# motionlife/gqmap-opticalflow

Hardware: AMD Instinct MI355X
Metric: Gpixel-iters/s + AEPE vs .flo GT, Middlebury 584x388, 1/2/4/8 GPU (higher is better)
Workload: dtype f64; 1 GPU; C2: rubberwhale 584x388 mixture L=1 K=9 its=2541 (one step = one full-frame iteration); engine=mixture, L=1, K=9, parallelism=frame-parallel x1

## Files before the change

gqmap-opticalflow_amd/csrc/gqmap_engine.hip:

```cpp
#include <dlfcn.h>
#include <hip/hip_runtime.h>
#include <rccl/rccl.h>

#include <algorithm>
#include <chrono>
#include <condition_variable>
#include <cstdlib>
#include <cmath>
#include <cstring>
#include <mutex>
#include <string>
#include <vector>

#include "gqmap_internal.h"
#include "gqmap_blockmatch.h"

#pragma clang fp contract(off)

namespace gq {
__device__ __forceinline__ double gq_sqrt_dev(double x)
{
    const double y = __builtin_amdgcn_rsq(x);
    double g = x * y, h = 0.5 * y;
    const double r = fma(-h, g, 0.5);
// ... 70 lines not shown
}
#define GQ_ROOT_STAGED 1

#define GQ_HD __device__ __forceinline__
#define GQ_SQRT(x) gq::gq_sqrt_dev(x)
#include "gqmap_tuning.h"
#define GQ_STR2(x) #x
#define GQ_PRAGMA_UNROLL(n) _Pragma(GQ_STR2(unroll n))
#define GQ_UNROLL2 GQ_PRAGMA_UNROLL(GQ_EDGE_UNROLL_N)
#define GQ_PAIR_UNROLL GQ_PRAGMA_UNROLL(GQ_PAIR_UNROLL_N)
#define GQ_PAIR_UNROLL_K(n) GQ_PRAGMA_UNROLL(n)
#define GQ_NODE_UNROLL GQ_PRAGMA_UNROLL(GQ_NODE_UNROLL_N)
#define GQ_UNROLL_FULL _Pragma("unroll")
#define GQ_UMUL24(a, b) __umul24((uint32_t)(a), (uint32_t)(b))
#define GQ_FRACT(x) __builtin_amdgcn_fract(x)
#include "gqmap_math.h"

namespace gq {

typedef float vvs_t;

constexpr int TILE = 16;
constexpr int BLOCK = TILE * TILE;
constexpr int TS = TAB_STRIDE;
constexpr int NPLANES = 9;
constexpr int TRACE_CAP = 8192;
constexpr int GRAPH_CHUNK = 50;
#ifndef GQ_FLOW_CHUNK
#define GQ_FLOW_CHUNK 250
#endif
// ... 589 lines not shown
        for (int x = 0; x < ACC_SLICES; ++x) t += v[x];
#pragma unroll
        for (int x = 0; x < ACC_SLICES; ++x) __hip_atomic_store(a + x * SL, 0ull, __ATOMIC_RELAXED, __HIP_MEMORY_SCOPE_AGENT);
        sh[tid] = t;
    }
    __syncthreads();
    if (tid < NP) {
        fix128 v = 0;
#pragma unroll
        for (int k = 3; k >= 0; --k) v = (v << 32) + (fix128)(long long)sh[4 * tid + k];
        out[tid] = v;
    }
    if (tid == 0) ctl->arrive = 0;
}

template <typename R, typename VT, int ENG, int Q, bool EDGE_FIRST, bool COH = false, bool NT = false,
          bool LIT = false, bool GRP = false, int ROTF = GQ_NODE_ROT_OTHER, int HALO = 0>
__device__ __forceinline__ void iter_tile(const IterParams<R, VT> P, int tile, int it, int parity,
                                          int part_r, TileLdsQ<R, Q> &lds, int l0, int l1, double Tcur,
                                          bool tab_ready, unsigned long long *acc_ring = nullptr,
                                          int grows = 0, bool grouped = false, HaloChain<R> *hc = nullptr,
                                          unsigned halo_tok = 0
#if GQ_FLOW_TL
                                          , unsigned long long *tlw = nullptr
#endif
                                          )
{
    static_assert(HALO == 0 || (GRP && sizeof(R) == 8), "the halo forms: the fp64 dataflow item (one component per item)");
    constexpr bool CHAIN = HALO == 1;
    static_assert(!LIT || (ENG == 0 && Q == 1 && sizeof(R) == 8), "literal order: fp64 mixture, Q = 1");
    static_assert(!GRP || (Q == 1 && !LIT), "a tile per wave: one lane per node");
    constexpr bool RS = Q == 0;
    constexpr int QA = arith_q(Q);
    constexpr int TPIX = tile_pix(Q);
    constexpr int TM = tile_rows(Q), TN = TPIX / TM;
    static_assert(TM * TN == TPIX, "tile");
    Ctl *ctl = P.ctl;
// ... 66 lines not shown
        R eE = 0, eda = 0;
#pragma unroll
        for (int ph = 0; ph < 2; ++ph) {
        if ((ph == 0) != EDGE_FIRST) {
        if (do_node && LIT) {
            if constexpr (LIT)
                if (inner)
                    nd = lit_node_grad(tab, K2, P.VV, P.M2, P.I1, P.Mo, P.No, P.epsn, P.lamd, P.guard != 0, T, a,
                                       mu_u, mu_v, sg_u, sg_v, pn, m, n + P.n_off);
        } else if (do_node) {
        NodeCoef<R> c{};
        if (inner) c = node_coef(sg_u, sg_v, pn);
        const bool fast = ENG == 0 && __all(!inner || node_unclamped(c, mu_u, mu_v, m, n + P.n_off, P.Mo, P.No,
                                                                     P.gh_xmax, R(ENG == 2 ? CTF_MARGIN : 0.0)));
        if (inner) {
            const auto fv = frame_view(P.VV, P.M2);
            constexpr bool PF = QA >= GQ_NODE_PF_MIN_Q && (QA > 1 || sizeof(VT) == 4);
            constexpr int ROT = PF ? ROTF : 0;
            Sums<R> S = fast ? node_sums<ENG, false, PF, ROT>(tab, kj, K2, QA, fv, P.I1, P.Mo, P.No, P.epsn, c, mu_u,
                                                              mu_v, m, n + P.n_off)
                             : node_sums<ENG, true, PF, ROT>(tab, kj, K2, QA, fv, P.I1, P.Mo, P.No, P.epsn, c, mu_u,
                                                             mu_v, m, n + P.n_off);
            if (QA > 1) S = lane_combine<QA>(S);
            nd = node_epi(S, c, P.lamd, P.guard != 0, T, a, sg_u, sg_v, pn, ENG == 2);
            if constexpr (RS) {
                lds.nd[0][pix] = nd.du1; lds.nd[1][pix] = nd.du2; lds.nd[2][pix] = nd.do1;
                lds.nd[3][pix] = nd.do2; lds.nd[4][pix] = nd.dp; lds.nd[5][pix] = nd.E; lds.nd[6][pix] = nd.da;
            }
        }
        }
        } else if (do_edge) {
// ... 685 lines not shown
void k_iter_flow(IterParams<R, VT> P, int n_iter, unsigned *fl, int ntiles, const Ctl *snap)
{
    static_assert(Q >= 1 && Q <= 4, "1..4 lanes per node");
    static_assert(!LIT || (ENG == 0 && Q == 1), "literal order: the mixture engine at one lane per node");
    unsigned *bar = P.bar;
    const bool run = !snap->stop && __hip_atomic_load(&P.ctl->stop, __ATOMIC_RELAXED, __HIP_MEMORY_SCOPE_AGENT) == 0 &&
                     __hip_atomic_load(bar + BAR_FAIL, __ATOMIC_RELAXED, __HIP_MEMORY_SCOPE_AGENT) == 0;
    const int it0 = snap->it, done0 = snap->done;
    const double T0 = snap->T;
    const int b = blockIdx.x, xcd = b & 7;
    int s0 = 0;
    for (int y = 0; y < xcd; ++y) s0 += (ntiles - y + 7) >> 3;
    const int nb = (ntiles - xcd + 7) >> 3;
    const int L = ENG == 1 ? P.L : 1, nitems = ntiles * L;
    constexpr bool GRP = GQ_FLOW_GROUPS && Q == 1 && !LIT && (ENG == 0 || ENG == 2);
    constexpr int ROTF = ENG == 0 && Q == 1 && !LIT && W == 0 && sizeof(R) == 8 && is_vvh2<VT>::value
                             ? (GQ_NODE_ROT_FLOW_FP64 | NODE_UNROLL(GQ_NODE_UNROLL_FLOW_FP64))
                             : GQ_NODE_ROT_OTHER;
    constexpr int HALO = !GRP || LIT || W != 0 || sizeof(R) != 8 ? 0
                         : ENG == 0 && is_vvh2<VT>::value ? GQ_FLOW_HALO
                         : ENG == 2 ? GQ_FLOW_HALO_CTF : 0;
    HaloChain<R> *hc = nullptr;
    if constexpr (HALO == 1) {
        __shared__ HaloChain<R> sh_halo;
        hc = &sh_halo;
        if (threadIdx.x < 4) sh_halo.flag[threadIdx.x] = 0;
        if (threadIdx.x == 0) sh_halo.fail = bar + BAR_FAIL;
    }
    const int vr = P.M - (P.tiles_m - 1) * tile_rows(Q);
    const bool groups = GRP && GQ_FLOW_ROWS && vr <= 4;
    const int nlast = groups ? (s0 + nb) / P.tiles_m - s0 / P.tiles_m : 0;
    const int nbl = groups ? nb - nlast + ((nlast + 3) >> 2) : nb * L;
    constexpr int INV = ENG == 2 && Q == 1 ? GQ_PHASE_MIX_CTF_Q1_INV : GQ_PHASE_MIX_OTHER_INV;
    constexpr bool MIX = GQ_FLOW_MIX && ENG == 0 && (!LIT || GQ_FLOW_LIT_MIX);
    const bool edge_first = MIX && ((((b >> 3) / P.cu_slots) & 1) != INV);
    __shared__ TileLdsQ<R, Q> lds;
    __shared__ int sh_i, sh_go, sh_last;
    __shared__ int sh_grp[4];
    __shared__ double tot[NFIX + GQMAP_LMAX];
    __shared__ unsigned long long sh_acc[4 * (NFIX + GQMAP_LMAX)];
    unsigned long long *acc = reinterpret_cast<unsigned long long *>(fl + FL_ACC);
    unsigned *q = fl + FL_Q + xcd * FL_LINE;
// ... 46 lines not shown
            for (int q = 0; q < nd; ++q) T = fmax(T * P.fin.drate, P.fin.t_min);
        }
        unsigned long long *slot = acc + (size_t)(j % FL_SLOTS) * FL_ACC_SLOT;
        const int l0 = ENG == 1 ? l : 0, l1 = ENG == 1 ? l + 1 : 1;
        const int wtile = GRP ? __builtin_amdgcn_readfirstlane(grouped ? sh_grp[threadIdx.x >> 6] : tile) : tile;
        const int wrows = grouped ? vr : tile_rows(Q);
#if GQ_FLOW_TL
        const size_t tlwi = (size_t)j * nitems + (size_t)tile * L + l;
        unsigned long long *tlw = (tlwi + 1) * 16 <= (size_t)(4 * FLOW_TL_WORDS) && snap->it == 1 ? g_flow_tlw + tlwi * 16 : nullptr;
#define GQ_TLW_ARG , tlw
#else
#define GQ_TLW_ARG
#endif
        if (MIX && edge_first)
            iter_tile<R, VT, ENG, Q, true, GQ_FLOW_COH, false, LIT, GRP, ROTF, HALO>(P, wtile, it, parity, 0, lds, l0, l1, T, false, slot,
                                                                                wrows, grouped, hc, (unsigned)i + 1 GQ_TLW_ARG);
        else
            iter_tile<R, VT, ENG, Q, false, GQ_FLOW_COH, false, LIT, GRP, ROTF, HALO>(P, wtile, it, parity, 0, lds, l0, l1, T, false, slot,
                                                                                 wrows, grouped, hc, (unsigned)i + 1 GQ_TLW_ARG);
#undef GQ_TLW_ARG
        asm volatile("s_waitcnt vmcnt(0)" ::: "memory");
        __syncthreads();
#if GQ_FLOW_TL
        const size_t tli = (size_t)j * nitems + (size_t)tile * L + l;
        if (threadIdx.x == 0 && (tli + 1) * 4 <= (size_t)FLOW_TL_WORDS && snap->it == 1) {
            unsigned long long *w = g_flow_tl + tli * 4;
            w[0] = tl_claim;
            w[1] = tl_go;
            w[2] = __builtin_amdgcn_s_memrealtime();
            w[3] = ((unsigned long long)__builtin_amdgcn_s_getreg((31 << 11) | 20) << 32) |
                   (unsigned)__builtin_amdgcn_s_getreg((31 << 11) | 4);
        }
#endif
        if (GRP && grouped && threadIdx.x > 0 && (int)threadIdx.x < gsize)
// ... 302 lines not shown

namespace gq {
struct Policy {
    int nt_state = -1;
    int band_rows = -1;
    int cu_group = -1;
    int lpar = -1;
    int lpar_xcd = 1;
    int fused_finalize = 1;
    int persist = 1;
    int persist_cap = -1;
    int graph = 1;
    int flow = -1;
    int vv_float = 1;
    int vv_pair = 1;
    int verbose = 0;
};
Policy g_pol;
}

struct gqmap_ctx {
    gqmap_options opt;
    int device = 0;
    hipStream_t stream = nullptr;
    bool fp32 = false, super_ = false;
    int Mo = 0, No = 0, M = 0, N = 0, L = 0, K = 0, K2 = 0;
    int64_t MNL = 0;
    size_t rsz = 8;
    void *d_VV = nullptr, *d_I1 = nullptr, *d_st[2] = {nullptr, nullptr}, *d_tab = nullptr;
    Ctl *d_ctl = nullptr;
// ... 3 lines not shown
    Ctl *d_snap_ctl = nullptr;
    size_t snap_bytes = 0;
    bool persist_off = false;
    double *d_trace = nullptr;
    Ctl *h_ctl = nullptr;
    double *h_ring = nullptr;
    unsigned *h_fail = nullptr;
    int ctl_it = 0;
    bool ctl_known = false;
    double *d_truth = nullptr;
    size_t truth_elems = 0;
    int tiles_m = 0, tiles_n = 0, nblocks = 0;
    bool have_images = false, have_state = false;
    bool vv32 = false;
    bool vvp = false;
    bool lit = false;
    int split = 1;
    int kq = 1;
    int lpar = 1;
    hipGraphExec_t graph = nullptr;
    hipGraphExec_t sub[6] = {nullptr, nullptr, nullptr, nullptr, nullptr, nullptr};
    bool own_stream = true;
    double tab_host[NTAB * TS];
    int n_tiles = 1, tile = 0, Ng = 0, col0 = 0, col1 = 0, n_off = 0, own_lo = 0, own_hi = 0;
    int nranks = 0;
    fix128 *d_gathered = nullptr;
    bool own_gathered = false;
    void *d_halo[4] = {nullptr, nullptr, nullptr, nullptr};
    struct RcclComm *comm = nullptr;
    bool in_group = false;
// ... 127 lines not shown
    if (c->pol.band_rows >= 0) return c->pol.band_rows == 1;
    const size_t vsz = c->fp32 ? sizeof(float) : c->vvp ? sizeof(vvh2_t) : c->vv32 ? sizeof(vvs_t) : sizeof(double);
    return vv_elems(c->Mo, c->No) * vsz > ((size_t)4 << 20);
}

bool fused_finalize(const gqmap_ctx *c)
{
    return c->nranks == 0 && c->pol.fused_finalize;
}

template <typename R, typename VT>
IterParams<R, VT> iter_params(const gqmap_ctx *c)
{
    IterParams<R, VT> P;
    const gqmap_options &o = c->opt;
    P.VV = (const VT *)c->d_VV;
    P.I1 = (const R *)c->d_I1;
    P.st0 = (R *)c->d_st[0];
    P.st1 = (R *)c->d_st[1];
    P.tab = (const R *)c->d_tab;
    P.ctl = c->d_ctl;
    P.partials = c->d_partials;
    P.M = c->M; P.N = c->N; P.Mo = c->Mo; P.No = c->No; P.M2 = c->Mo + 2;
    P.L = c->L; P.K2 = c->K2;
    P.tiles_m = c->tiles_m; P.tiles_n = c->tiles_n;
    P.seg_lo[0] = P.seg_lo[1] = 0;
    P.seg_n[0] = c->tiles_m * c->tiles_n;
    P.seg_n[1] = 0;
    P.part_off = 0;
    P.epsn = R(o.epsn); P.lamd = R(o.lambdad); P.lams = R(o.lambdas);
    P.minu = R(o.minu); P.maxu = R(o.maxu); P.minv = R(o.minv); P.maxv = R(o.maxv);
// ... 692 lines not shown
        }
        if (hipMemsetAsync(c->d_flow, 0, sizeof(unsigned) * flow_words(nitems), c->stream) != hipSuccess ||
            hipStreamSynchronize(c->stream) != hipSuccess)
            return false;
        c->flow_n = flow_words(nitems);
    }
    if (!ensure_snap(c)) return false;
    if (dry) return true;
    {
        const int64_t nv = (int64_t)c->MNL * NPLANES;
        const int grid = (int)std::min<int64_t>((nv + 255) / 256, 512);
        k_persist_snap<R><<<grid, 256, 0, c->stream>>>(c->d_ctl, c->d_bar, (const R *)c->d_st[0],
                                                       (const R *)c->d_st[1], (R *)c->d_snap, c->d_snap_ctl, nv);
    }
    IterParams<R, VT> P = iter_params<R, VT>(c);
    if constexpr (ENG == 0 && Q == 1 && !LIT) {
        if (nitems > GQ_FLOW_WIDE_ITEMS) {
            flow_launch<R, VT, ENG, Q, LIT, 3>(c, P, n, nitems, ntiles);
            return true;
        }
    }
    flow_launch<R, VT, ENG, Q, LIT, 0>(c, P, n, nitems, ntiles);
    return true;
}

template <typename R, typename VT>
bool launch_flow_t(gqmap_ctx *c, int n, bool dry)
{
    if (c->opt.engine == GQMAP_ENGINE_SUPER) {
        if constexpr (sizeof(R) == 8) return c->pol.flow > 0 && c->kq == 4 && launch_flow_q<R, VT, 1, 4>(c, n, dry);
        return false;
// ... 13 lines not shown
        default: return false;
        }
    }
    return false;
}

bool launch_flow(gqmap_ctx *c, int n, bool dry)
{
    const bool on = c->pol.flow > 0 || (c->pol.flow < 0 && !c->fp32);
    if (!on || c->persist_off || (c->L != 1 && c->opt.engine != GQMAP_ENGINE_SUPER) || c->n_tiles != 1 ||
        c->comm || c->nranks != 0 || !fused_finalize(c) || n < 1)
        return false;
    if (c->fp32)
        return c->vvp ? !c->lit && c->kq == 1 && launch_flow_q<float, vvh2_t, 0, 1>(c, n, dry)
                      : launch_flow_t<float, float>(c, n, dry);
    if (c->vvp) return !c->lit && c->kq == 1 && launch_flow_q<double, vvh2_t, 0, 1>(c, n, dry);
    if (c->vv32) return launch_flow_t<double, vvs_t>(c, n, dry);
    return launch_flow_t<double, double>(c, n, dry);
}

gqmap_status persist_recover(gqmap_ctx *c, bool *recovered)
{
    *recovered = false;
    if (!c->d_snap) return GQMAP_OK;
    c->ctl_known = false;
    unsigned f = 0;
    GQ_HIP(hipMemcpyAsync(&f, c->d_bar + BAR_FAIL, sizeof(f), hipMemcpyDeviceToHost, c->stream));
    GQ_HIP(hipStreamSynchronize(c->stream));
    if (f == 0) return GQMAP_OK;
    Ctl h;
// ... 174 lines not shown
    strip_geometry(c, Mo, No);
    tile_grid(c);
    if (vvp && (c->kq != 1 || c->split != 1)) {
        vvp = false;
        vv32 = true;
    }
    const bool resize = geom || vv32 != c->vv32 || vvp != c->vvp || !c->d_VV;
    c->vv32 = vv32;
    c->vvp = vvp;
    if (resize) {
        drop_graph(c);
        GQ_HIP(hipStreamSynchronize(c->stream));
        if (c->d_VV) (void)hipFree(c->d_VV);
        if (c->d_I1) (void)hipFree(c->d_I1);
        c->d_VV = c->d_I1 = nullptr;
        if (c->d_truth) (void)hipFree(c->d_truth);
        c->d_truth = nullptr;
        c->truth_elems = 0;
        const size_t vsz = c->fp32 ? sizeof(float) : vvp ? sizeof(vvh2_t) : vv32 ? sizeof(vvs_t) : sizeof(double);
        GQ_HIP(hipMalloc(&c->d_VV, vv_elems(Mo, No) * vsz));
        GQ_HIP(hipMemsetAsync(c->d_VV, 0, vv_elems(Mo, No) * vsz, c->stream));
        GQ_HIP(hipMalloc(&c->d_I1, (size_t)Mo * No * c->rsz));
        gqmap_status s = alloc_grid(c);
        if (s != GQMAP_OK) return s;
        c->have_state = false;
        if (c->n_tiles > 1) {
            for (int k = 0; k < 4; ++k) {
                if (c->d_halo[k]) (void)hipFree(c->d_halo[k]);
                c->d_halo[k] = nullptr;
                GQ_HIP(hipMalloc(&c->d_halo[k], halo_bytes(c, k)));
// ... 244 lines not shown
    gqmap_status s = prepare_images(c, Mo, No, vv32, vvp);
    if (s != GQMAP_OK) return s;
    vvp = c->vvp;
    vv32 = c->vv32;
    DeviceGuard dg(c->device);
    if (vvp) {
        const size_t M2 = (size_t)Mo + 2, N2 = (size_t)No + 2;
        std::vector<vvh2_t> vp(VV.size());
        for (size_t cc = 0; cc < N2; ++cc)
            for (size_t r = 0; r < M2; ++r) {
                vp[r + M2 * cc].lo = (_Float16)VV[r + M2 * cc];
                vp[r + M2 * cc].hi = cc + 1 < N2 ? (_Float16)VV[r + M2 * (cc + 1)] : (_Float16)0;
            }
        GQ_HIP(hipMemcpyAsync(c->d_VV, vp.data(), vp.size() * sizeof(vvh2_t), hipMemcpyHostToDevice, c->stream));
        GQ_HIP(hipStreamSynchronize(c->stream));
    } else if (vv32 && !c->fp32) {
        std::vector<vvs_t> vc(VV.size());
        for (size_t k = 0; k < VV.size(); ++k) vc[k] = (vvs_t)VV[k];
        GQ_HIP(hipMemcpyAsync(c->d_VV, vc.data(), vc.size() * sizeof(vvs_t), hipMemcpyHostToDevice, c->stream));
        GQ_HIP(hipStreamSynchronize(c->stream));
    } else if (vv32) {
        std::vector<float> v32(VV.begin(), VV.end());
        GQ_HIP(hipMemcpyAsync(c->d_VV, v32.data(), v32.size() * sizeof(float), hipMemcpyHostToDevice, c->stream));
        GQ_HIP(hipStreamSynchronize(c->stream));
    } else if ((s = upload(c, c->d_VV, VV.data(), VV.size())) != GQMAP_OK) {
        return s;
    }
    if ((s = upload(c, c->d_I1, I1, (size_t)Mo * No)) != GQMAP_OK) return s;
    c->have_images = true;
    return GQMAP_OK;
// ... 453 lines not shown
}

int gqmap_debug_flow_chunk(void) { return FLOW_CHUNK; }

int gqmap_debug_policy(const char *name, int value)
{
    if (!name) return -1;
    struct Field { const char *n; int *p; int dflt; };
    const Field fields[] = {
        {"nt_state", &g_pol.nt_state, -1},   {"band_rows", &g_pol.band_rows, -1},
        {"cu_group", &g_pol.cu_group, -1},   {"lpar", &g_pol.lpar, -1},
        {"lpar_xcd", &g_pol.lpar_xcd, 1},    {"fused_finalize", &g_pol.fused_finalize, 1},
        {"persist", &g_pol.persist, 1},      {"persist_cap", &g_pol.persist_cap, -1},
        {"graph", &g_pol.graph, 1},          {"vv_float", &g_pol.vv_float, 1}, {"vv_pair", &g_pol.vv_pair, 1},
        {"verbose", &g_pol.verbose, 0},      {"flow", &g_pol.flow, -1},
    };
    for (const Field &f : fields)
        if (std::strcmp(f.n, name) == 0) {
            *f.p = value == -1 ? f.dflt : value;
            return 0;
        }
    return -1;
}

gqmap_status gqmap_get_info(gqmap_ctx *c, gqmap_info *info)
{
    clear_error();
    GQ_CHECK(c && info, GQMAP_ERR_INVALID_ARG, "null argument");
    DeviceGuard dg(c->device);
    std::memset(info, 0, sizeof(*info));
// ... 125 lines not shown
        GQ_HIP(hipMemcpyAsync(out, c->d_VV, nvv * sizeof(double), hipMemcpyDeviceToHost, c->stream));
        GQ_HIP(hipStreamSynchronize(c->stream));
        return GQMAP_OK;
    }
    const size_t esz = c->fp32 ? sizeof(float) : sizeof(vvs_t);
    std::vector<unsigned char> raw(nvv * esz);
    GQ_HIP(hipMemcpyAsync(raw.data(), c->d_VV, raw.size(), hipMemcpyDeviceToHost, c->stream));
    GQ_HIP(hipStreamSynchronize(c->stream));
    for (size_t k = 0; k < nvv; ++k) {
        if (c->fp32) out[k] = ((const float *)raw.data())[k];
        else out[k] = (double)((const vvs_t *)raw.data())[k];
    }
    return GQMAP_OK;
}

gqmap_status gqmap_synchronize(gqmap_ctx *c)
{
    clear_error();
    GQ_CHECK(c, GQMAP_ERR_INVALID_ARG, "null context");
    DeviceGuard dg(c->device);
    GQ_HIP(hipStreamSynchronize(c->stream));
    return GQMAP_OK;
}

gqmap_status gqmap_create_tile(gqmap_ctx **out, const gqmap_options *opt, int device, int n_tiles, int tile)
{
    clear_error();
    GQ_CHECK(n_tiles >= 1 && n_tiles <= 1024, GQMAP_ERR_INVALID_ARG, "n_tiles=%d outside [1,1024]", n_tiles);
    GQ_CHECK(tile >= 0 && tile < n_tiles, GQMAP_ERR_INVALID_ARG, "tile %d of %d", tile, n_tiles);
    gqmap_status s = gqmap_create(out, opt, device);
// ... 282 lines not shown
void gqmap_destroy(gqmap_ctx *c)
{
    if (!c) return;
    DeviceGuard dg(c->device);
    if (c->stream) (void)hipStreamSynchronize(c->stream);
    drop_graph(c);
    if (c->comm) {
        if (c->comm->comm) (void)rccl()->CommDestroy(c->comm->comm);
        delete c->comm;
    }
    for (void *p : {(void *)c->d_rows, (void *)c->d_seqg})
        if (p) (void)hipFree(p);
    if (c->own_gathered && c->d_gathered) (void)hipFree(c->d_gathered);
    for (void *p : c->d_halo)
        if (p) (void)hipFree(p);
    void *bufs[] = {c->d_VV, c->d_I1, c->d_st[0], c->d_st[1], c->d_tab, c->d_ctl, (void *)c->d_partials, c->d_trace,
                    c->d_truth, (void *)c->d_bar, c->d_snap, (void *)c->d_snap_ctl, (void *)c->d_flow};
    for (void *p : bufs)
        if (p) (void)hipFree(p);
    for (void *p : {(void *)c->h_ctl, (void *)c->h_ring, (void *)c->h_fail})
        if (p) (void)hipHostFree(p);
    if (c->stream && c->own_stream) (void)hipStreamDestroy(c->stream);
    delete c;
}

}
```

gqmap-opticalflow_amd/csrc/gqmap_math.h:

```cpp
#pragma once
#include <stdint.h>
#include <string.h>

#include <type_traits>

namespace gq {

#ifndef GQ_M_PI
#define GQ_M_PI 3.14159265358979323846
#define GQ_M_SQRT2 1.41421356237309504880
#endif

constexpr int TAB_STRIDE = 256;
constexpr int NTAB = 8;
constexpr int T_XI = 0, T_XJ = 1, T_W = 2, T_WA = 3, T_WXI = 4, T_WXJ = 5, T_WM = 6, T_WX = 7;
#ifdef __HIPCC__
__host__ __device__
#endif
constexpr int tab_at(int r, int k) { return k * NTAB + r; }

GQ_HD uint64_t bits_of(double x)
{
    uint64_t u;
    memcpy(&u, &x, 8);
// ... 120 lines not shown
GQ_HD VP elem_ptr(VP VV, uint32_t elem)
{
    return byte_ptr(VV, elem * (uint32_t)sizeof(*VV));
}

#if defined(__HIPCC__)
struct alignas(4) vvh2_t {
    _Float16 lo, hi;
};
template <typename T>
struct is_vvh2 : std::is_same<typename std::remove_cv<T>::type, vvh2_t> {};
#else
template <typename T>
struct is_vvh2 : std::false_type {};
#endif
template <typename R, typename E>
GQ_HD R tap_col(const E &e, int half)
{
#if defined(__HIPCC__)
    if constexpr (is_vvh2<E>::value) return R((float)(half ? e.hi : e.lo));
    else
#endif
    {
        (void)half;
        return R(e);
    }
}

template <typename R, typename VP>
GQ_HD R bicubic_w4(VP VV, uint32_t o, uint32_t M2, R s0, R s1, R s2, R s3, R t0, R t1, R t2, R t3)
// ... 30 lines not shown
    keys4(so, s0, s1, s2, s3);
    return bicubic_w4<R>(VV, o, M2, s0, s1, s2, s3, t0, t1, t2, t3);
}

template <typename E>
struct Taps16 {
    E v[16];
};
template <typename VP>
GQ_HD auto load_taps16(VP VV, uint32_t o, uint32_t M2)
{
    using E = typename std::remove_cv<typename std::remove_reference<decltype(*VV)>::type>::type;
    constexpr uint32_t EB = (uint32_t)sizeof(E);
    const uint32_t ob = o * EB, cb = M2 * EB;
    Taps16<E> T;
    if constexpr (is_vvh2<E>::value) {
        for (int pr = 0; pr < 2; ++pr) {
            const auto col = byte_ptr(VV, ob + (uint32_t)(2 * pr) * cb);
            for (int r = 0; r < 4; ++r) T.v[4 * pr + r] = col[r];
        }
        return T;
    } else {
        for (int c = 0; c < 4; ++c) {
            const auto col = byte_ptr(VV, ob + (uint32_t)c * cb);
            for (int r = 0; r < 4; ++r) T.v[4 * c + r] = col[r];
        }
        return T;
    }
}
template <typename R, typename E>
GQ_HD R bicubic_taps4(const Taps16<E> &T, R so, R to)
// ... 47 lines not shown
    return fma(s3, v[3], fma(s2, v[2], fma(s1, v[1], s0 * v[0])));
}

GQ_HD uint32_t cell_elem(int iy, int ix, int M2) { return (uint32_t)(iy - 1) + GQ_UMUL24(M2, ix - 1); }

template <typename VP>
struct TapView {
    VP p;
    uint32_t ld;
    GQ_HD uint32_t cell(int iy, int ix) const { return cell_elem(iy, ix, (int)ld); }
};
template <typename VP>
GQ_HD TapView<VP> frame_view(VP VV, int M2)
{
    return TapView<VP>{VV, (uint32_t)M2};
}

constexpr int VV_TAIL = 8;
constexpr size_t vv_elems(int Mo, int No) { return (size_t)(Mo + 2) * (size_t)(No + 3) + VV_TAIL; }

template <bool CLAMP = true>
GQ_HD void axis_cell_abs(double X, int n, int &ix, double &fr)
{
    if (CLAMP) X = fmin(fmax(X, 1.0), (double)n);
    ix = (int)X;
    fr = GQ_FRACT(X);
}
template <bool CLAMP = true>
GQ_HD void axis_cell(int j, double x, int n, int &ix, double &fr)
{
// ... 372 lines not shown
    R s, t, ax, bx, ay, by;
};
template <typename R>
GQ_HD NodeCoef<R> node_coef(R o1, R o2, R p)
{
    NodeCoef<R> c;
    spectral_st(p, c.s, c.t);
    const R sq2 = R(GQ_M_SQRT2);
    c.ax = sq2 * o1 * c.s; c.bx = sq2 * o1 * c.t;
    c.ay = sq2 * o2 * c.t; c.by = sq2 * o2 * c.s;
    return c;
}
constexpr int NODE_ROT = 1, NODE_ROT_STAGE = 2, NODE_ROT_FLAGS = 255;
constexpr int NODE_UNROLL(int n) { return n << 8; }
constexpr int node_rot_unroll(int rot) { return (rot >> 8) > 1 ? (rot >> 8) : 1; }
template <int ENG, bool CLAMP = true, bool PF = false, int ROT = 0, typename R, typename TP, typename TV, typename IP>
GQ_HD Sums<R> node_sums(TP tab, int k0, int K2, int dk, const TV &V, IP I1, int Mo, int No,
                        R eps, const NodeCoef<R> &c, R u1, R u2, int m, int n)
{
    Sums<R> S;
    if constexpr (PF && ENG != 1) {
        const R I = I1[m + (int64_t)Mo * n];
        constexpr bool ABS = ENG == 0 && sizeof(R) == 8;
        const R U1 = ABS ? u1 + R(n + 1) : u1, U2 = ABS ? u2 + R(m + 1) : u2;
        auto locate = [&](int k, R &so, R &to) -> uint32_t {
            const R x1 = fma(c.ax, tab[tab_at(T_XI, k)], fma(c.bx, tab[tab_at(T_XJ, k)], U1));
            const R x2 = fma(c.ay, tab[tab_at(T_XI, k)], fma(c.by, tab[tab_at(T_XJ, k)], U2));
            if constexpr (ABS) return cell4_abs_v<CLAMP>(V, Mo, No, (double)x1, (double)x2, so, to);
            else if constexpr (ENG == 2) return cell_ctf4_v<CLAMP>(V, Mo, No, m + 1, n + 1, x1, x2, so, to);
            else return cell4_v<CLAMP>(V, Mo, No, m + 1, n + 1, x1, x2, so, to);
        };
        if constexpr ((ROT & NODE_ROT_FLAGS) != 0) {
            static_assert(ROT & NODE_ROT, "the other bits modify the rotated loop");
            constexpr bool STAGE = (ROT & NODE_ROT_STAGE) != 0;
            constexpr int UNR = node_rot_unroll(ROT);
            (void)UNR;
// ... 30 lines not shown
            R so, to;
            auto T = load_taps16(V.p, locate(k0, so, to), V.ld);
            constexpr int UNR = node_rot_unroll(ROT);
            (void)UNR;
            GQ_PAIR_UNROLL_K(UNR)
            for (int k = k0; k <= klast; k += dk) {
                const auto Tk = T;
                const R sok = so, tok = to;
                const int kn = k + dk <= klast ? k + dk : klast;
                T = load_taps16(V.p, locate(kn, so, to), V.ld);
                const R d = fma(bicubic_taps4<R>(Tk, sok, tok), R(-0.25), I);
                S.add(tab, k, GQ_SQRT(fma(d, d, eps)));
            }
        }
        return S;
    }
    if constexpr (ENG != 1) {
        const R I = I1[m + (int64_t)Mo * n];
        if constexpr (ENG == 0 && sizeof(R) == 8) {
            const R U1 = u1 + R(n + 1), U2 = u2 + R(m + 1);
            GQ_NODE_UNROLL
            for (int k = k0; k < K2; k += dk) {
                const R X = fma(c.ax, tab[tab_at(T_XI, k)], fma(c.bx, tab[tab_at(T_XJ, k)], U1));
                const R Y = fma(c.ay, tab[tab_at(T_XI, k)], fma(c.by, tab[tab_at(T_XJ, k)], U2));
                const R d = fma(sample4_abs_v<CLAMP>(V, Mo, No, X, Y), R(-0.25), I);
                S.add(tab, k, GQ_SQRT(fma(d, d, eps)));
            }
        } else {
            GQ_NODE_UNROLL
            for (int k = k0; k < K2; k += dk) {
                const R x1 = fma(c.ax, tab[tab_at(T_XI, k)], fma(c.bx, tab[tab_at(T_XJ, k)], u1));
                const R x2 = fma(c.ay, tab[tab_at(T_XI, k)], fma(c.by, tab[tab_at(T_XJ, k)], u2));
// ... 424 lines not shown
```

gqmap-opticalflow_amd/csrc/gqmap_tuning.h:

```cpp
#pragma once

#ifndef GQ_EDGE_UNROLL_N
#define GQ_EDGE_UNROLL_N 2
#endif
#ifndef GQ_PAIR_UNROLL_N
#define GQ_PAIR_UNROLL_N 2
#endif
#ifndef GQ_PAIR_UNROLL_Q1
#define GQ_PAIR_UNROLL_Q1 4
#endif
#ifndef GQ_NODE_UNROLL_N
#define GQ_NODE_UNROLL_N 1
#endif
#ifndef GQ_FIN_GROUP
#define GQ_FIN_GROUP 1
#endif
#ifndef GQ_EDGE_PK
#define GQ_EDGE_PK 1
#endif
#ifndef GQ_TAB_LDS
#define GQ_TAB_LDS 1
#endif
#ifndef GQ_PHASE_MIX
#define GQ_PHASE_MIX 1
// ... 31 lines not shown
#ifndef GQ_FLOW_HALO
#define GQ_FLOW_HALO 1
#endif
#ifndef GQ_FLOW_HALO_CTF
#define GQ_FLOW_HALO_CTF 1
#endif
#ifndef GQ_FLOW_HALO_ROT_WAVE
#define GQ_FLOW_HALO_ROT_WAVE 2
#endif
#ifndef GQ_FLOW_HALO_EPI
#define GQ_FLOW_HALO_EPI 8
#endif
#ifndef GQ_FLOW_HALO_SLEEP
#define GQ_FLOW_HALO_SLEEP 1
#endif
#ifndef GQ_UNROLL_MIN_Q
#define GQ_UNROLL_MIN_Q 2
#endif
#ifndef GQ_PERSIST_Q4
#define GQ_PERSIST_Q4 0
#endif
#ifndef GQ_PERSIST_SLEEP
#define GQ_PERSIST_SLEEP 2
#endif
#ifndef GQ_TIMELINE
#define GQ_TIMELINE 0
#endif
```

Before: 1.788 Gpixel-iter/s.

## Store frame taps as 16-bit LDS offsets into a per-block value LUT

When the frame pixel values are integers within a small range, the flow kernel stores each tap as a uint16 byte offset into a shared-memory table of doubles instead of half-precision pairs. Each bicubic tap is then resolved by an LDS load, and a dedicated pipelined node-sum loop uses scheduling fences and register pins to overlap the next tap fetch with the current arithmetic. The aim is to reduce the cost of tap fetch and conversion in the fp64 mixture node loop. In exchange it adds per-block LUT fill, extra LDS pressure, a second device buffer and host preprocessing, and it disables the wide-item variant on this path.

```diff
diff --git a/gqmap-opticalflow_amd/csrc/gqmap_engine.hip b/gqmap-opticalflow_amd/csrc/gqmap_engine.hip
--- a/gqmap-opticalflow_amd/csrc/gqmap_engine.hip
+++ b/gqmap-opticalflow_amd/csrc/gqmap_engine.hip
@@ -108,6 +108,11 @@
 #define GQ_UNROLL_FULL _Pragma("unroll")
 #define GQ_UMUL24(a, b) __umul24((uint32_t)(a), (uint32_t)(b))
 #define GQ_FRACT(x) __builtin_amdgcn_fract(x)
+#define GQ_LDS_AS __attribute__((address_space(3)))
+#define GQ_LUT_AT(lut, o) (*(const GQ_LDS_AS double *)((const GQ_LDS_AS char *)(lut) + (o)))
+#define GQ_SCHED_FENCE __builtin_amdgcn_sched_barrier(0)
+#define GQ_PIN64(x) asm volatile("" : "+v"(x))
+#define GQ_PIN_UNIFORM(x) asm volatile("" : "+s"(x))
 #include "gqmap_math.h"
 
 namespace gq {
@@ -727,13 +732,24 @@
     if (tid == 0) ctl->arrive = 0;
 }
 
+template <typename R, typename VT>
+__device__ __forceinline__ auto tile_frame_view(const IterParams<R, VT> &P, const GQ_LDS_AS double *taplut)
+{
+    if constexpr (is_vvo2<VT>::value) {
+        return frame_view_lut(P.VV, P.M2, taplut);
+    } else {
+        (void)taplut;
+        return frame_view(P.VV, P.M2);
+    }
+}
+
 template <typename R, typename VT, int ENG, int Q, bool EDGE_FIRST, bool COH = false, bool NT = false,
           bool LIT = false, bool GRP = false, int ROTF = GQ_NODE_ROT_OTHER, int HALO = 0>
 __device__ __forceinline__ void iter_tile(const IterParams<R, VT> P, int tile, int it, int parity,
                                           int part_r, TileLdsQ<R, Q> &lds, int l0, int l1, double Tcur,
                                           bool tab_ready, unsigned long long *acc_ring = nullptr,
                                           int grows = 0, bool grouped = false, HaloChain<R> *hc = nullptr,
-                                          unsigned halo_tok = 0
+                                          unsigned halo_tok = 0, const GQ_LDS_AS double *taplut = nullptr
 #if GQ_FLOW_TL
                                           , unsigned long long *tlw = nullptr
 #endif
@@ -830,7 +846,7 @@
         const bool fast = ENG == 0 && __all(!inner || node_unclamped(c, mu_u, mu_v, m, n + P.n_off, P.Mo, P.No,
                                                                      P.gh_xmax, R(ENG == 2 ? CTF_MARGIN : 0.0)));
         if (inner) {
-            const auto fv = frame_view(P.VV, P.M2);
+            const auto fv = tile_frame_view(P, taplut);
             constexpr bool PF = QA >= GQ_NODE_PF_MIN_Q && (QA > 1 || sizeof(VT) == 4);
             constexpr int ROT = PF ? ROTF : 0;
             Sums<R> S = fast ? node_sums<ENG, false, PF, ROT>(tab, kj, K2, QA, fv, P.I1, P.Mo, P.No, P.epsn, c, mu_u,
@@ -1546,11 +1562,11 @@
     const int nb = (ntiles - xcd + 7) >> 3;
     const int L = ENG == 1 ? P.L : 1, nitems = ntiles * L;
     constexpr bool GRP = GQ_FLOW_GROUPS && Q == 1 && !LIT && (ENG == 0 || ENG == 2);
-    constexpr int ROTF = ENG == 0 && Q == 1 && !LIT && W == 0 && sizeof(R) == 8 && is_vvh2<VT>::value
-                             ? (GQ_NODE_ROT_FLOW_FP64 | NODE_UNROLL(GQ_NODE_UNROLL_FLOW_FP64))
+    constexpr int ROTF = ENG == 0 && Q == 1 && !LIT && W == 0 && sizeof(R) == 8 && is_vvpair<VT>::value
+                             ? ((is_vvo2<VT>::value ? 0 : GQ_NODE_ROT_FLOW_FP64) | NODE_UNROLL(GQ_NODE_UNROLL_FLOW_FP64))
                              : GQ_NODE_ROT_OTHER;
     constexpr int HALO = !GRP || LIT || W != 0 || sizeof(R) != 8 ? 0
-                         : ENG == 0 && is_vvh2<VT>::value ? GQ_FLOW_HALO
+                         : ENG == 0 && is_vvpair<VT>::value ? GQ_FLOW_HALO
                          : ENG == 2 ? GQ_FLOW_HALO_CTF : 0;
     HaloChain<R> *hc = nullptr;
     if constexpr (HALO == 1) {
@@ -1558,6 +1574,14 @@
         hc = &sh_halo;
         if (threadIdx.x < 4) sh_halo.flag[threadIdx.x] = 0;
         if (threadIdx.x == 0) sh_halo.fail = bar + BAR_FAIL;
+    }
+    const GQ_LDS_AS double *taplut = nullptr;
+    if constexpr (is_vvo2<VT>::value) {
+        __shared__ double sh_taplut[TAPLUT_N];
+        const int *hdr = reinterpret_cast<const int *>(P.VV + vv_elems(P.Mo, P.No));
+        const int vmin = hdr[0], vn = min(hdr[1], TAPLUT_N);
+        for (int e = threadIdx.x; e < vn; e += BLOCK) sh_taplut[e] = taplut_entry(e, vmin);
+        taplut = (const GQ_LDS_AS double *)sh_taplut;
     }
     const int vr = P.M - (P.tiles_m - 1) * tile_rows(Q);
     const bool groups = GRP && GQ_FLOW_ROWS && vr <= 4;
@@ -1634,10 +1658,10 @@
 #endif
         if (MIX && edge_first)
             iter_tile<R, VT, ENG, Q, true, GQ_FLOW_COH, false, LIT, GRP, ROTF, HALO>(P, wtile, it, parity, 0, lds, l0, l1, T, false, slot,
-                                                                                wrows, grouped, hc, (unsigned)i + 1 GQ_TLW_ARG);
+                                                                                wrows, grouped, hc, (unsigned)i + 1, taplut GQ_TLW_ARG);
         else
             iter_tile<R, VT, ENG, Q, false, GQ_FLOW_COH, false, LIT, GRP, ROTF, HALO>(P, wtile, it, parity, 0, lds, l0, l1, T, false, slot,
-                                                                                 wrows, grouped, hc, (unsigned)i + 1 GQ_TLW_ARG);
+                                                                                 wrows, grouped, hc, (unsigned)i + 1, taplut GQ_TLW_ARG);
 #undef GQ_TLW_ARG
         asm volatile("s_waitcnt vmcnt(0)" ::: "memory");
         __syncthreads();
@@ -1970,6 +1994,7 @@
     int flow = -1;
     int vv_float = 1;
     int vv_pair = 1;
+    int tap_lut = 1;
     int verbose = 0;
 };
 Policy g_pol;
@@ -2003,6 +2028,8 @@
     bool have_images = false, have_state = false;
     bool vv32 = false;
     bool vvp = false;
+    bool tapt = false;
+    void *d_VO = nullptr;
     bool lit = false;
     int split = 1;
     int kq = 1;
@@ -2160,7 +2187,7 @@
 {
     IterParams<R, VT> P;
     const gqmap_options &o = c->opt;
-    P.VV = (const VT *)c->d_VV;
+    P.VV = (const VT *)(is_vvo2<VT>::value ? c->d_VO : c->d_VV);
     P.I1 = (const R *)c->d_I1;
     P.st0 = (R *)c->d_st[0];
     P.st1 = (R *)c->d_st[1];
@@ -2883,7 +2910,7 @@
                                                        (const R *)c->d_st[1], (R *)c->d_snap, c->d_snap_ctl, nv);
     }
     IterParams<R, VT> P = iter_params<R, VT>(c);
-    if constexpr (ENG == 0 && Q == 1 && !LIT) {
+    if constexpr (ENG == 0 && Q == 1 && !LIT && !is_vvo2<VT>::value) {
         if (nitems > GQ_FLOW_WIDE_ITEMS) {
             flow_launch<R, VT, ENG, Q, LIT, 3>(c, P, n, nitems, ntiles);
             return true;
@@ -2927,6 +2954,10 @@
     if (c->fp32)
         return c->vvp ? !c->lit && c->kq == 1 && launch_flow_q<float, vvh2_t, 0, 1>(c, n, dry)
                       : launch_flow_t<float, float>(c, n, dry);
+#if GQ_TAP_LUT
+    if (c->vvp && c->tapt && c->tiles_m * c->tiles_n <= GQ_FLOW_WIDE_ITEMS)
+        return !c->lit && c->kq == 1 && launch_flow_q<double, vvo2_t, 0, 1>(c, n, dry);
+#endif
     if (c->vvp) return !c->lit && c->kq == 1 && launch_flow_q<double, vvh2_t, 0, 1>(c, n, dry);
     if (c->vv32) return launch_flow_t<double, vvs_t>(c, n, dry);
     return launch_flow_t<double, double>(c, n, dry);
@@ -3131,6 +3162,9 @@
         if (c->d_VV) (void)hipFree(c->d_VV);
         if (c->d_I1) (void)hipFree(c->d_I1);
         c->d_VV = c->d_I1 = nullptr;
+        if (c->d_VO) (void)hipFree(c->d_VO);
+        c->d_VO = nullptr;
+        c->tapt = false;
         if (c->d_truth) (void)hipFree(c->d_truth);
         c->d_truth = nullptr;
         c->truth_elems = 0;
@@ -3405,6 +3439,40 @@
             }
         GQ_HIP(hipMemcpyAsync(c->d_VV, vp.data(), vp.size() * sizeof(vvh2_t), hipMemcpyHostToDevice, c->stream));
         GQ_HIP(hipStreamSynchronize(c->stream));
+        bool tapt = GQ_TAP_LUT && c->pol.tap_lut && !c->fp32;
+        int vmin = 0, vmax = 0;
+        for (size_t k = 0; tapt && k < VV.size(); ++k) {
+            const int vi = (int)VV[k];
+            if ((double)vi != VV[k]) tapt = false;
+            vmin = std::min(vmin, vi);
+            vmax = std::max(vmax, vi);
+        }
+        if (tapt && vmax - vmin + 1 > TAPLUT_N) tapt = false;
+        if (tapt != c->tapt) drop_graph(c);
+        c->tapt = false;
+        if (tapt) {
+            struct Undo {
+                gqmap_ctx *c;
+                bool armed;
+                ~Undo() { if (armed) drop_graph(c); }
+            } undo{c, true};
+            const size_t ne = vv_elems(Mo, No);
+            if (!c->d_VO) GQ_HIP(hipMalloc(&c->d_VO, ne * sizeof(vvo2_t) + 2 * sizeof(int)));
+            const uint16_t zero = taplut_offset(0, vmin);
+            std::vector<vvo2_t> vo(ne + 2, vvo2_t{zero, zero});
+            for (size_t cc = 0; cc < N2; ++cc)
+                for (size_t r = 0; r < M2; ++r) {
+                    vo[r + M2 * cc].lo = taplut_offset((int)VV[r + M2 * cc], vmin);
+                    if (cc + 1 < N2) vo[r + M2 * cc].hi = taplut_offset((int)VV[r + M2 * (cc + 1)], vmin);
+                }
+            const int hdr[2] = {vmin, vmax - vmin + 1};
+            static_assert(sizeof(hdr) == 2 * sizeof(vvo2_t), "the two words behind the elements");
+            std::memcpy(&vo[ne], hdr, sizeof(hdr));
+            GQ_HIP(hipMemcpyAsync(c->d_VO, vo.data(), vo.size() * sizeof(vvo2_t), hipMemcpyHostToDevice, c->stream));
+            GQ_HIP(hipStreamSynchronize(c->stream));
+            c->tapt = true;
+            undo.armed = false;
+        }
     } else if (vv32 && !c->fp32) {
         std::vector<vvs_t> vc(VV.size());
         for (size_t k = 0; k < VV.size(); ++k) vc[k] = (vvs_t)VV[k];
@@ -3888,6 +3956,7 @@
         {"persist", &g_pol.persist, 1},      {"persist_cap", &g_pol.persist_cap, -1},
         {"graph", &g_pol.graph, 1},          {"vv_float", &g_pol.vv_float, 1}, {"vv_pair", &g_pol.vv_pair, 1},
         {"verbose", &g_pol.verbose, 0},      {"flow", &g_pol.flow, -1},
+        {"tap_lut", &g_pol.tap_lut, 1},
     };
     for (const Field &f : fields)
         if (std::strcmp(f.n, name) == 0) {
@@ -4043,6 +4112,41 @@
     return GQMAP_OK;
 }
 
+int gqmap_debug_tap_lut(const gqmap_ctx *c) { return c && c->have_images && c->vvp && c->tapt ? 1 : 0; }
+
+gqmap_status gqmap_debug_read_vo(gqmap_ctx *c, double *lo, double *hi, size_t n, int *tail, int range[2])
+{
+    clear_error();
+    GQ_CHECK(c && lo && hi && tail && range, GQMAP_ERR_INVALID_ARG, "null argument");
+    GQ_CHECK(c->have_images && c->vvp && c->tapt && c->d_VO, GQMAP_ERR_STATE, "no offset store");
+    const size_t nvv = (size_t)(c->Mo + 2) * (c->No + 2), ne = vv_elems(c->Mo, c->No);
+    GQ_CHECK(n >= nvv, GQMAP_ERR_INVALID_ARG, "buffer holds %zu of %zu values", n, nvv);
+    DeviceGuard dg(c->device);
+    std::vector<vvo2_t> raw(ne + 2);
+    GQ_HIP(hipMemcpyAsync(raw.data(), c->d_VO, raw.size() * sizeof(vvo2_t), hipMemcpyDeviceToHost, c->stream));
+    GQ_HIP(hipStreamSynchronize(c->stream));
+    std::memcpy(range, &raw[ne], 2 * sizeof(int));
+    auto value = [&](uint16_t o) { return o % 8 == 0 && o / 8 < range[1] ? taplut_entry(o / 8, range[0]) : (double)NAN; };
+    for (size_t k = 0; k < nvv; ++k) {
+        lo[k] = value(raw[k].lo);
+        hi[k] = value(raw[k].hi);
+    }
+    *tail = 0;
+    for (size_t k = nvv; k < ne; ++k) *tail += (value(raw[k].lo) != 0.0) + (value(raw[k].hi) != 0.0);
+    return GQMAP_OK;
+}
+
+int gqmap_debug_flow_per_cu(gqmap_ctx *c)
+{
+    if (!c || !c->have_images || !c->vvp || c->fp32) return -1;
+    DeviceGuard dg(c->device);
+    if (c->tiles_m * c->tiles_n > GQ_FLOW_WIDE_ITEMS) return kernel_shape(k_iter_flow<double, vvh2_t, 0, 1, false, 3>).x;
+#if GQ_TAP_LUT
+    if (c->tapt) return kernel_shape(k_iter_flow<double, vvo2_t, 0, 1, false, 0>).x;
+#endif
+    return kernel_shape(k_iter_flow<double, vvh2_t, 0, 1, false, 0>).x;
+}
+
 gqmap_status gqmap_synchronize(gqmap_ctx *c)
 {
     clear_error();
@@ -4355,7 +4459,7 @@
     if (c->own_gathered && c->d_gathered) (void)hipFree(c->d_gathered);
     for (void *p : c->d_halo)
         if (p) (void)hipFree(p);
-    void *bufs[] = {c->d_VV, c->d_I1, c->d_st[0], c->d_st[1], c->d_tab, c->d_ctl, (void *)c->d_partials, c->d_trace,
+    void *bufs[] = {c->d_VV, c->d_VO, c->d_I1, c->d_st[0], c->d_st[1], c->d_tab, c->d_ctl, (void *)c->d_partials, c->d_trace,
                     c->d_truth, (void *)c->d_bar, c->d_snap, (void *)c->d_snap_ctl, (void *)c->d_flow};
     for (void *p : bufs)
         if (p) (void)hipFree(p);
diff --git a/gqmap-opticalflow_amd/csrc/gqmap_math.h b/gqmap-opticalflow_amd/csrc/gqmap_math.h
--- a/gqmap-opticalflow_amd/csrc/gqmap_math.h
+++ b/gqmap-opticalflow_amd/csrc/gqmap_math.h
@@ -158,6 +158,26 @@
 template <typename T>
 struct is_vvh2 : std::false_type {};
 #endif
+constexpr int TAPLUT_N = 1276;
+struct alignas(4) vvo2_t {
+    uint16_t lo, hi;
+};
+template <typename T>
+struct is_vvo2 : std::is_same<typename std::remove_cv<T>::type, vvo2_t> {};
+template <typename T>
+struct is_vvpair : std::integral_constant<bool, is_vvh2<T>::value || is_vvo2<T>::value> {};
+#ifdef __HIPCC__
+__host__ __device__
+#endif
+constexpr uint16_t taplut_offset(int value, int vmin) { return (uint16_t)((value - vmin) * 8); }
+#ifdef __HIPCC__
+__host__ __device__
+#endif
+constexpr double taplut_entry(int i, int vmin) { return (double)(vmin + i); }
+#ifndef GQ_LUT_AT
+#define GQ_LUT_AT(lut, o) (*(const double *)((const char *)(lut) + (o)))
+#endif
+
 template <typename R, typename E>
 GQ_HD R tap_col(const E &e, int half)
 {
@@ -218,7 +238,7 @@
     constexpr uint32_t EB = (uint32_t)sizeof(E);
     const uint32_t ob = o * EB, cb = M2 * EB;
     Taps16<E> T;
-    if constexpr (is_vvh2<E>::value) {
+    if constexpr (is_vvpair<E>::value) {
         for (int pr = 0; pr < 2; ++pr) {
             const auto col = byte_ptr(VV, ob + (uint32_t)(2 * pr) * cb);
             for (int r = 0; r < 4; ++r) T.v[4 * pr + r] = col[r];
@@ -296,6 +316,30 @@
 GQ_HD TapView<VP> frame_view(VP VV, int M2)
 {
     return TapView<VP>{VV, (uint32_t)M2};
+}
+template <typename VP, typename LP>
+struct TapViewLut {
+    VP p;
+    uint32_t ld;
+    LP lut;
+    GQ_HD uint32_t cell(int iy, int ix) const { return cell_elem(iy, ix, (int)ld); }
+};
+template <typename VP, typename LP>
+GQ_HD TapViewLut<VP, LP> frame_view_lut(VP VV, int M2, LP lut)
+{
+    return TapViewLut<VP, LP>{VV, (uint32_t)M2, lut};
+}
+template <typename LP>
+GQ_HD Taps16<double> lut_taps16(LP lut, const Taps16<vvo2_t> &T, uint32_t mask = 0xffffu, uint32_t shift = 16)
+{
+    Taps16<double> D;
+    for (int c = 0; c < 4; ++c)
+        for (int r = 0; r < 4; ++r) {
+            const vvo2_t &e = T.v[4 * (c >> 1) + r];
+            const uint32_t w = (uint32_t)e.lo | (uint32_t)e.hi << 16;
+            D.v[4 * c + r] = GQ_LUT_AT(lut, (c & 1) ? w >> shift : w & mask);
+        }
+    return D;
 }
 
 constexpr int VV_TAIL = 8;
@@ -698,12 +742,71 @@
 constexpr int NODE_ROT = 1, NODE_ROT_STAGE = 2, NODE_ROT_FLAGS = 255;
 constexpr int NODE_UNROLL(int n) { return n << 8; }
 constexpr int node_rot_unroll(int rot) { return (rot >> 8) > 1 ? (rot >> 8) : 1; }
+#ifndef GQ_SCHED_FENCE
+#define GQ_SCHED_FENCE (void)0
+#define GQ_PIN64(x) (void)(x)
+#define GQ_PIN_UNIFORM(x) (void)(x)
+#endif
+template <bool CLAMP, int UNR, typename TP, typename TV, typename IP>
+GQ_HD Sums<double> node_sums_lut(TP tab, int k0, int K2, int dk, const TV &V, IP I1, int Mo, int No, double eps,
+                                 const NodeCoef<double> &c, double u1, double u2, int m, int n)
+{
+    Sums<double> S;
+    if (k0 >= K2) return S;
+    const double I = I1[m + (int64_t)Mo * n];
+    const double U1 = u1 + double(n + 1), U2 = u2 + double(m + 1);
+    auto locate = [&](double xi, double xj, double &so, double &to) -> uint32_t {
+        const double x1 = fma(c.ax, xi, fma(c.bx, xj, U1));
+        const double x2 = fma(c.ay, xi, fma(c.by, xj, U2));
+        return cell4_abs_v<CLAMP>(V, Mo, No, x1, x2, so, to);
+    };
+    const int klast = k0 + (K2 - 1 - k0) / dk * dk;
+    double so, to;
+    auto T = load_taps16(V.p, locate(tab[tab_at(T_XI, k0)], tab[tab_at(T_XJ, k0)], so, to), V.ld);
+    const int kn0 = k0 + dk <= klast ? k0 + dk : klast;
+    double nxi = tab[tab_at(T_XI, kn0)], nxj = tab[tab_at(T_XJ, kn0)];
+    auto trip = [&](int k) {
+        uint32_t mask = 0xffffu, shift = 16;
+        GQ_PIN_UNIFORM(mask);
+        GQ_PIN_UNIFORM(shift);
+        const Taps16<double> D = lut_taps16(V.lut, T, mask, shift);
+        GQ_SCHED_FENCE;
+        double sok = so, tok = to;
+        T = load_taps16(V.p, locate(nxi, nxj, so, to), V.ld);
+        GQ_SCHED_FENCE;
+        GQ_PIN64(sok);
+        GQ_PIN64(tok);
+        const int kn2 = k + 2 * dk <= klast ? k + 2 * dk : klast;
+        nxi = tab[tab_at(T_XI, kn2)];
+        nxj = tab[tab_at(T_XJ, kn2)];
+        const double d = fma(bicubic_taps4<double>(D, sok, tok), -0.25, I);
+        S.add(tab, k, GQ_SQRT(fma(d, d, eps)));
+        GQ_PIN64(S.s0); GQ_PIN64(S.sxi); GQ_PIN64(S.sxj);
+        GQ_PIN64(S.sa); GQ_PIN64(S.sm); GQ_PIN64(S.sx);
+        GQ_SCHED_FENCE;
+    };
+    int k = k0;
+    GQ_PAIR_UNROLL_K(1)
+    for (; k + (UNR - 1) * dk <= klast; k += UNR * dk) {
+        GQ_UNROLL_FULL
+        for (int u = 0; u < UNR; ++u) trip(k + u * dk);
+    }
+    if constexpr (UNR > 1) {
+        GQ_PAIR_UNROLL_K(1)
+        for (; k <= klast; k += dk) trip(k);
+    }
+    return S;
+}
 template <int ENG, bool CLAMP = true, bool PF = false, int ROT = 0, typename R, typename TP, typename TV, typename IP>
 GQ_HD Sums<R> node_sums(TP tab, int k0, int K2, int dk, const TV &V, IP I1, int Mo, int No,
                         R eps, const NodeCoef<R> &c, R u1, R u2, int m, int n)
 {
     Sums<R> S;
-    if constexpr (PF && ENG != 1) {
+    if constexpr (is_vvo2<typename std::remove_cv<typename std::remove_reference<decltype(*V.p)>::type>::type>::value) {
+        static_assert(PF && ENG == 0 && sizeof(R) == 8 && (ROT & NODE_ROT_FLAGS) == 0,
+                      "the offset store: the fp64 single-scale engine's pipelined loop, not rotated");
+        return node_sums_lut<CLAMP, node_rot_unroll(ROT)>(tab, k0, K2, dk, V, I1, Mo, No, eps, c, u1, u2, m, n);
+    } else if constexpr (PF && ENG != 1) {
         const R I = I1[m + (int64_t)Mo * n];
         constexpr bool ABS = ENG == 0 && sizeof(R) == 8;
         const R U1 = ABS ? u1 + R(n + 1) : u1, U2 = ABS ? u2 + R(m + 1) : u2;
@@ -764,8 +867,7 @@
             }
         }
         return S;
-    }
-    if constexpr (ENG != 1) {
+    } else if constexpr (ENG != 1) {
         const R I = I1[m + (int64_t)Mo * n];
         if constexpr (ENG == 0 && sizeof(R) == 8) {
             const R U1 = u1 + R(n + 1), U2 = u2 + R(m + 1);
diff --git a/gqmap-opticalflow_amd/csrc/gqmap_tuning.h b/gqmap-opticalflow_amd/csrc/gqmap_tuning.h
--- a/gqmap-opticalflow_amd/csrc/gqmap_tuning.h
+++ b/gqmap-opticalflow_amd/csrc/gqmap_tuning.h
@@ -69,6 +69,9 @@
 #ifndef GQ_FLOW_HALO_SLEEP
 #define GQ_FLOW_HALO_SLEEP 1
 #endif
+#ifndef GQ_TAP_LUT
+#define GQ_TAP_LUT 1
+#endif
 #ifndef GQ_UNROLL_MIN_Q
 #define GQ_UNROLL_MIN_Q 2
 #endif
```

New measurement: 1.868 Gpixel-iter/s, median of 6. 4.4% higher.
